# nonl4331/raytracing-rust

Measured on AMD Instinct MI355X. Metric: Msamples/s on rtweekend1.ssml 1920x1080x1024spp, higher is better.
Workload: dtype f32

## Files before the change

include/rt_hip.h:

```cpp
#ifndef RT_HIP_H
#define RT_HIP_H

#include <stdint.h>

#ifdef __cplusplus
extern "C" {
#endif

#define RT_ABI_VERSION 2u

typedef enum rt_status {
	RT_OK = 0,
	RT_ERR_INVALID_ARGUMENT = -1,
	RT_ERR_NO_DEVICE = -2,
	RT_ERR_HIP = -3,
	RT_ERR_OUT_OF_MEMORY = -4,
	RT_ERR_UNSUPPORTED = -5
} rt_status;

typedef enum rt_texture_type {
	RT_TEX_CHECKERED = 0,
	RT_TEX_SOLID = 1,
	RT_TEX_IMAGE = 2,
	RT_TEX_LERP = 3,
// ... 332 lines not shown
	float metered;
	uint32_t reserved;
} rt_display_state;
int rt_display_opts_default(rt_display_opts *out);
int rt_display_workspace_bytes(const rt_display_opts *opts, uint64_t *bytes);
int rt_display_output_bytes(const rt_display_opts *opts, uint64_t *bytes);
int rt_display_device(rt_scene *scene, const float *d_rgb, const rt_display_opts *opts, rt_display_state *d_state,
                      void *d_workspace, void *d_out, uint32_t *d_histogram, void *hip_stream);
int rt_display(rt_scene *scene, const float *host_rgb, const rt_display_opts *opts, void *host_out, rt_display_state *host_state,
               uint32_t *host_histogram);
int rt_display_reset(rt_scene *scene);

typedef struct rt_upscale_opts {
	uint32_t src_width, src_height;
	uint32_t dst_width, dst_height;
	float sigma_normal;
	float depth_tolerance;
	uint32_t reserved[8];
} rt_upscale_opts;
typedef struct rt_upscale_inputs {
	const float *color;
	const float *src_albedo, *src_normal, *src_depth;
	const float *dst_albedo, *dst_normal, *dst_depth;
} rt_upscale_inputs;
int rt_upscale_opts_default(rt_upscale_opts *out);
int rt_upscale_device(rt_scene *scene, const rt_upscale_inputs *device_in, const rt_upscale_opts *opts, float *d_out, uint8_t *d_stage,
                      void *hip_stream);
int rt_upscale(rt_scene *scene, const rt_upscale_inputs *host_in, const rt_upscale_opts *opts, float *host_out, uint8_t *host_stage);
int rt_render_upscaled(rt_scene *scene, const rt_camera *camera, const rt_render_opts *opts, uint32_t src_width, uint32_t src_height,
                       const rt_denoise_opts *dopts, const rt_upscale_opts *uopts, float *out, float *out_src, uint64_t *rays_shot);

int rt_selftest_division(float divisor, float *reciprocal, int *exact);

#define RT_SELFTEST_LEAN_CLASSES 9
int rt_selftest_lean(int device, uint64_t n_per_thread, uint64_t seed, uint64_t mismatches[RT_SELFTEST_LEAN_CLASSES]);

#ifdef __cplusplus
}
#endif
#endif
```

raytracing-rust_amd/abi.py:

```python
import ctypes as C

RT_ABI_VERSION = 2
RT_GATHER_NONE, RT_GATHER_RCCL, RT_GATHER_PEER, RT_GATHER_PEER_STAGED, RT_GATHER_SAME_DEVICE = 0, 1, 2, 3, 4

RT_OK = 0
RT_ERR_INVALID_ARGUMENT = -1
RT_ERR_NO_DEVICE = -2
RT_ERR_HIP = -3
RT_ERR_OUT_OF_MEMORY = -4
RT_ERR_UNSUPPORTED = -5

RT_TEX_CHECKERED, RT_TEX_SOLID, RT_TEX_IMAGE, RT_TEX_LERP, RT_TEX_PERLIN = range(5)
RT_MAT_EMIT, RT_MAT_LAMBERTIAN, RT_MAT_TROWBRIDGE_REITZ, RT_MAT_REFLECT, RT_MAT_REFRACT = range(5)
RT_PRIM_SPHERE, RT_PRIM_TRIANGLE, RT_PRIM_MESH_TRIANGLE = range(3)
RT_SPLIT_SAH, RT_SPLIT_MIDDLE, RT_SPLIT_EQUAL_COUNTS = range(3)
RT_METHOD_NAIVE, RT_METHOD_MIS = range(2)
RT_LAYOUT_FRAME, RT_LAYOUT_SHARD = range(2)
RT_TUNE_TRAVERSAL, RT_TUNE_FEATURE_SET, RT_TUNE_SCENE_IN_LDS, RT_TUNE_SCHEDULE, RT_TUNE_WALK, RT_TUNE_STACK_CAP, RT_TUNE_EXCHANGE = range(7)

NO_INDEX = 0xFFFFFFFFFFFFFFFF
RT_DEVICE_NONE = -1

f32x3 = C.c_float * 3

# ... 331 lines not shown
    "rt_aov_chain_buffers": (AovChainBuffers, 56),
    "rt_denoise_opts": (DenoiseOpts, 48),
    "rt_denoise_inputs": (DenoiseInputs, 40),
    "rt_temporal_opts": (TemporalOpts, 96),
    "rt_temporal_inputs": (TemporalInputs, 32),
    "rt_display_opts": (DisplayOpts, 104),
    "rt_display_state": (DisplayState, 16),
    "rt_upscale_opts": (UpscaleOpts, 56),
    "rt_upscale_inputs": (UpscaleInputs, 56),
}

EXPORTED_SYMBOLS = [
    "rt_last_error",
    "rt_abi_version",
    "rt_device_count",
    "rt_render_opts_default",
    "rt_camera_new",
    "rt_scene_create",
    "rt_scene_create_multi",
    "rt_scene_device_count",
    "rt_scene_destroy",
    "rt_scene_counts",
    "rt_scene_get_nodes",
    "rt_scene_get_primitive_order",
    "rt_scene_get_lights",
    "rt_scene_wide_info",
    "rt_scene_get_wide_nodes",
    "rt_scene_get_leaf_boxes",
    "rt_scene_get_wide_nodes_compact",
    "rt_scene_auto_sample_split",
    "rt_scene_gather_info",
    "rt_rccl_probe",
    "rt_selftest_division",
    "rt_scene_get_leaf_boxes_compact",
    "rt_scene_set_traversal",
    "rt_scene_set_tuning",
    "rt_render",
    "rt_sample_image",
    "rt_render_device",
    "rt_render_output_floats",
    "rt_shard_pixel_order",
    "rt_last_kernel_ms",
    "rt_last_launch_info",
    "rt_output_rgb8",
    "rt_output_save",
    "rt_output_rgb8_device",
    "rt_render_rgb8",
    "rt_check_hit",
    "rt_check_hit_index",
    "rt_selftest_lean",
    "rt_render_aov",
    "rt_render_aov_device",
    "rt_aov_chain_opts_default",
    "rt_render_aov_chain",
    "rt_render_aov_chain_device",
    "rt_denoise_opts_default",
    "rt_denoise_workspace_bytes",
    "rt_denoise",
    "rt_denoise_device",
    "rt_render_denoised",
    "rt_temporal_opts_default",
    "rt_temporal_history_bytes",
    "rt_temporal_workspace_bytes",
    "rt_denoise_temporal_device",
    "rt_denoise_temporal",
    "rt_denoise_temporal_reset",
# ... 42 lines not shown
```

raytracing-rust_amd/csrc/rt_api.cpp:

```cpp
#include <hip/hip_runtime.h>

#include <cstdio>
#include <cstdlib>
#include <algorithm>
#include <cmath>
#include <cstring>
#include <string>
#include <vector>

#include "../../include/rt_hip.h"
#include "../../include/rt_detmath.h"
#include <dlfcn.h>
#include "rt_api_internal.h"

namespace rt {
size_t render_lds_bytes(const DevScene &S, bool sky_lds, bool scene_lds, uint32_t waves_per_block, uint32_t stack_cap);
uint32_t render_waves_per_simd(int feature_set, bool fine);
uint32_t render_block_threads(int feature_set, bool fine, bool xchg = false);
size_t render_exchange_fine_lds_bytes(uint32_t waves_per_block);
uint32_t render_max_block_threads(int feature_set, bool fine, bool xchg);
hipError_t render_occupancy(int method, bool prune, bool fine, bool sky_lds, int feature_set, size_t lds_bytes, int *blocks_per_cu, bool xchg,
                            uint32_t block_threads = 0);
bool render_exchange_available(int method, bool prune, bool fine, int feature_set);
size_t render_exchange_lds_bytes(uint32_t slots);
// ... 1036 lines not shown
			return fail(RT_ERR_NO_DEVICE, "host-only scene");
		return render_device_multi(s, camera, o, d_out_rgb, d_rays_shot, static_cast<hipStream_t>(hip_stream));
	}
	ShardGeometry g;
	int rc = shard_geometry(o, g);
	if (rc != RT_OK)
		return rc;
	if (s->device == RT_DEVICE_NONE)
		return fail(RT_ERR_NO_DEVICE, "host-only scene (RT_DEVICE_NONE): rendering needs a GPU, there is no CPU fallback");
	if (o->render_method != RT_METHOD_NAIVE && o->render_method != RT_METHOD_MIS)
		return fail(RT_ERR_INVALID_ARGUMENT, "unknown render method");
	if (o->samples_per_pixel == 0 || o->samples_per_pixel >= (1ull << 32))
		return fail(RT_ERR_INVALID_ARGUMENT, "samples_per_pixel must be in [1, 2^32)");
	if (o->output_layout != RT_LAYOUT_FRAME && o->output_layout != RT_LAYOUT_SHARD)
		return fail(RT_ERR_INVALID_ARGUMENT, "unknown output layout");
	HIP_TRY(hipSetDevice(s->device));
	hipStream_t stream = static_cast<hipStream_t>(hip_stream);
	if (g.n_work == 0) {
		HIP_TRY(launch_reset(stream, s->d_work_counter, reinterpret_cast<unsigned long long *>(d_rays_shot), d_out_rgb,
		                     o->output_layout == RT_LAYOUT_FRAME ? (size_t)(o->width * o->height * 3) : 0));
		s->timed = false;
		return RT_OK;
	}

	DevRenderParams P;
	std::memset(&P, 0, sizeof P);
	P.width = (uint32_t)o->width;
	P.height = (uint32_t)o->height;
	P.spp = (uint32_t)o->samples_per_pixel;
	P.sample_begin_lo = (uint32_t)o->sample_begin;
	P.sample_begin_hi = (uint32_t)(o->sample_begin >> 32);
	P.seed_lo = (uint32_t)o->seed;
	P.seed_hi = (uint32_t)(o->seed >> 32);
	P.max_depth = o->max_depth;
	P.rr_threshold = o->rr_threshold;
	P.shard_index = o->shard_index;
	P.shard_count = o->shard_count;
	P.tile_w = g.tile_w;
	P.tile_h = g.tile_h;
	P.tiles_x = g.tiles_x;
	P.tiles_y = g.tiles_y;
	P.n_work = (uint32_t)g.n_work;
	uint32_t split = o->sample_split;
	if (split == 0u)
		split = auto_sample_split(s->n_cus, o->width * o->height, o->samples_per_pixel, o->shard_count);
	{
		float rw = 0.0f, rh = 0.0f;
		const bool sized = o->width <= (1u << 24) && o->height <= (1u << 24);
		const bool ok_w = sized && verified_reciprocal((float)(o->width - 1), &rw), ok_h = sized && verified_reciprocal((float)(o->height - 1), &rh);
		const bool ok = ok_w && ok_h;
		P.w1h1_ok = ok ? 1u : 0u;
		P.inv_w1 = rw;
		P.inv_h1 = rh;
	}
	P.tile_log2_w = 0xFFFFFFFFu;
	if (g.tile_w * g.tile_h == 64u && (g.tile_w & (g.tile_w - 1u)) == 0u && o->width < 65536u && o->height < 65536u &&
	    (split & (split - 1u)) == 0u && split <= 64u)
		for (uint32_t lw = 0; lw < 7u; ++lw)
			for (uint32_t ls = 0; ls < 7u; ++ls)
				if ((1u << lw) == g.tile_w && (1u << ls) == split)
					P.tile_log2_w = lw | (ls << 8);
	if (split > o->samples_per_pixel)
		return fail(RT_ERR_INVALID_ARGUMENT, "sample_split larger than samples_per_pixel");
	if (g.n_work * split >= (1ull << 32))
		return fail(RT_ERR_UNSUPPORTED, "pixels x sample_split exceeds 2^32 work items");
	P.sample_split = split;
// ... 645 lines not shown
	DevScene dev = s->dev;
	const bool walks_wide = prune && dev.nodes4 != nullptr && dev.narrow_only == 0u;
	if (!walks_wide || (size_t)4 * dev.stack_depth * 64u * sizeof(uint32_t) > s->max_lds) {
		if (walks_wide)
			dev.narrow_only = 1u;
		dev.stack_depth = s->stack_depth_narrow;
	}
	if (e == hipSuccess)
		e = object_index ? launch_check_hit_index(prune, s->stream, dev, d_rays, d_idx, n, d_out)
		                 : launch_check_hit(prune, s->stream, dev, d_rays, n, d_out);
	if (e == hipSuccess)
		e = hipMemcpyAsync(out, d_out, n * sizeof(rt_hit_record), hipMemcpyDeviceToHost, s->stream);
	if (e == hipSuccess)
		e = hipStreamSynchronize(s->stream);
	(void)hipFree(d_rays);
	(void)hipFree(d_out);
	(void)hipFree(d_idx);
	if (e != hipSuccess)
		return hip_fail(e, "check_hit");
	return RT_OK;
}

int rt_check_hit(rt_scene *s, const rt_ray_desc *rays, uint64_t n_rays, rt_hit_record *out)
{
	return check_common(s, rays, nullptr, n_rays, out);
}
int rt_check_hit_index(rt_scene *s, const rt_ray_desc *rays, const uint64_t *object_index, uint64_t n_rays, rt_hit_record *out)
{
	if (!object_index)
		return fail(RT_ERR_INVALID_ARGUMENT, "null argument");
	return check_common(s, rays, object_index, n_rays, out);
}

int rt_selftest_division(float divisor, float *reciprocal, int *exact)
{
	if (!reciprocal || !exact)
		return fail(RT_ERR_INVALID_ARGUMENT, "null argument");
	*exact = verified_reciprocal(divisor, reciprocal) ? 1 : 0;
	return RT_OK;
}

int rt_selftest_lean(int device, uint64_t n_per_thread, uint64_t seed, uint64_t mismatches[RT_SELFTEST_LEAN_CLASSES])
{
	if (!mismatches || n_per_thread == 0 || n_per_thread > (1ull << 20))
		return fail(RT_ERR_INVALID_ARGUMENT, "bad arguments (n_per_thread in [1, 2^20])");
	int n_dev = 0;
	if (hipGetDeviceCount(&n_dev) != hipSuccess || device < 0 || device >= n_dev)
		return fail(RT_ERR_NO_DEVICE, "no such HIP device");
	HIP_TRY(hipSetDevice(device));
	unsigned long long *d = nullptr;
	HIP_TRY(hipMalloc(reinterpret_cast<void **>(&d), RT_SELFTEST_LEAN_CLASSES * sizeof(unsigned long long)));
	hipError_t e = hipMemset(d, 0, RT_SELFTEST_LEAN_CLASSES * sizeof(unsigned long long));
	if (e == hipSuccess)
		e = launch_selftest_lean(nullptr, 1024u, n_per_thread, seed, d);
	if (e == hipSuccess)
		e = hipMemcpy(mismatches, d, RT_SELFTEST_LEAN_CLASSES * sizeof(unsigned long long), hipMemcpyDeviceToHost);
	(void)hipFree(d);
	if (e != hipSuccess)
		return hip_fail(e, "selftest");
	return RT_OK;
}

}
```

raytracing-rust_amd/csrc/rt_lean.h:

```cpp
#pragma once

#include "rt_vec.h"

namespace rt {


RT_FN void lean_sincos(float x, float &s, float &c)
{
	const float k = rintf(x * 0.636619746685028076172f);
	float r = fmaf(-k, 1.57079637050628662109f, x);
	r = fmaf(-k, -4.37113882867379282984e-08f, r);
	r = fmaf(-k, -1.71512451000588185479e-15f, r);
	const int q = (int)k;
	const float sk = rt_sin_kernel(r), ck = rt_cos_kernel(r);
	const bool odd = (q & 1) != 0;
	const float sv = odd ? ck : sk;
	const float cv = odd ? sk : ck;
	s = (q & 2) ? -sv : sv;
	c = ((q + 1) & 2) ? -cv : cv;
}

RT_FN float lean_acos_with(float x, float sqrt_half_one_minus_abs)
{
	const bool big = fabsf(x) > 0.5f;
	const float k = rt_asin_kernel(big ? sqrt_half_one_minus_abs : x);
	const float two_k = 2.0f * k;
	return big ? (x > 0.0f ? two_k : RT_PI - two_k) : RT_FRAC_PI_2 - k;
}
RT_FN float lean_acos(float x) { return lean_acos_with(x, sqrtf(0.5f * (1.0f - fabsf(x)))); }

RT_FN float lean_atan_unit_with(float t, float q)
{
	const bool upper = t > 0.414213567972183227539f;
	const float u = upper ? q : t;
	const float z = u * u;
	float p = fmaf(8.05374449538e-2f, z, -1.38776856032e-1f);
	p = fmaf(p, z, 1.99777106478e-1f);
	p = fmaf(p, z, -3.33329491539e-1f);
// ... 104 lines not shown
```

raytracing-rust_amd/csrc/rt_render.hip:

```cpp
#include "rt_shade.h"

namespace rt {

enum : int {
	PH_GEN = 0,
	PH_NODE = 1,
	PH_LEAF = 2,
	PH_SHADE = 3,
	PH_LIGHT = 4,
	PH_SCATTER = 5,
	PH_NARROW = 6,
	PH_COUNT = 7,
	PH_NEED_PIXEL = 7,
	PH_DONE = 8,
	PH_WALK = 9
};

#ifndef RT_PQ_SPLIT
#define RT_PQ_SPLIT 1
#endif
#ifndef RT_LIGHT_PHASE_THRESHOLD
#define RT_LIGHT_PHASE_THRESHOLD 48
#endif
constexpr uint32_t kLightPhaseThreshold = RT_LIGHT_PHASE_THRESHOLD;
// ... 31 lines not shown
#define RT_SIMPLE_COARSE_WAVES 5
#endif
#ifndef RT_SIMPLE_COARSE_BLOCK
#define RT_SIMPLE_COARSE_BLOCK 256
#endif
#ifndef RT_SPHERES_BLOCK
#define RT_SPHERES_BLOCK 512
#endif
#ifndef RT_FUSE_REGIONS
#define RT_FUSE_REGIONS(spheres_only) true
#endif
#ifndef RT_BODY_ALWAYS
#define RT_BODY_ALWAYS(spheres_only) true
#endif
#ifndef RT_SPHERES_MAX_BLOCK
#define RT_SPHERES_MAX_BLOCK 768
#endif
#ifndef RT_PAIR_WAVES
#define RT_PAIR_WAVES 6
#endif
#ifndef RT_SPHERES_WAVES
#define RT_SPHERES_WAVES 4
#endif
#ifndef RT_SPHERES_COARSE_WAVES
#define RT_SPHERES_COARSE_WAVES 6
#endif

__device__ __forceinline__ float power_heuristic(float pdf_a, float pdf_b)
{
	const float a_sq = pdf_a * pdf_a;
	return a_sq / (a_sq + pdf_b * pdf_b);
}

__device__ __forceinline__ bool work_to_pixel(const DevRenderParams &P, uint32_t w, uint32_t &x, uint32_t &y)
{
	const uint32_t tile_pixels = P.tile_w * P.tile_h;
	const uint32_t k = w / tile_pixels;
	const uint32_t in = w - k * tile_pixels;
	const uint32_t tile = P.shard_index + k * P.shard_count;
	const uint32_t ty = tile / P.tiles_x;
	const uint32_t tx = tile - ty * P.tiles_x;
	x = tx * P.tile_w + in % P.tile_w;
	y = ty * P.tile_h + in / P.tile_w;
	return x < P.width && y < P.height;
}

template <class F, bool FINE = false, bool XCHG = false> struct KernelShape {
	static constexpr bool spheres_only = !(F::tri || F::lights || F::cmat || F::ctex);
	static constexpr bool simple = !spheres_only && !(F::cmat || F::ctex);
	static constexpr int waves_per_simd = (F::cmat || F::ctex) ? (FINE ? RT_FULL_FINE_WAVES : (XCHG ? 3 : RT_FULL_WAVES))
	                                      : (F::pair ? RT_PAIR_WAVES : (spheres_only ? ((FINE || XCHG) ? RT_SPHERES_WAVES : RT_SPHERES_COARSE_WAVES)
	                                                                                 : (FINE ? RT_SIMPLE_FINE_WAVES : (XCHG ? 4 : RT_SIMPLE_COARSE_WAVES))));
	static constexpr int block = (FINE && XCHG) ? 512 : (spheres_only ? RT_SPHERES_BLOCK : ((simple && !FINE) ? RT_SIMPLE_COARSE_BLOCK : 256));
	static constexpr int max_block = ((spheres_only || simple) && !FINE && !XCHG && block == 512) ? RT_SPHERES_MAX_BLOCK : block;
};

#ifdef RT_STATS
#define RT_SECTION(k) do { const unsigned long long now_ = wall_clock64(); st_sect[(k)] += now_ - st_mark; st_mark = now_; } while (0)
#else
#define RT_SECTION(k) do { } while (0)
#endif
#ifdef RT_STATS
__device__ unsigned long long g_stats[64];
__device__ unsigned long long g_hist[4][65];
#endif

constexpr uint32_t kXchgBStride = 44, kXchgPStride = 12;
constexpr uint32_t kXchgMaxSlots = 64;
constexpr uint32_t kXchgMinLanes = 4;
constexpr uint32_t kXchgRecWords = 60;
constexpr uint32_t kXchgFineSlots = 64;
constexpr uint32_t kXchgFineHdr = 8 + 2 * 64;
#ifndef RT_XCHG_SHADERS
#define RT_XCHG_SHADERS 1
#endif
constexpr uint32_t kXchgShaderWaves = RT_XCHG_SHADERS;
enum : uint32_t { XS_EMPTY = 0, XS_FULL = 1, XS_BUSY = 2 };

struct RenderArgs {
	DevScene S;
	DevCamera cam;
	DevRenderParams P;
	float *out;
	unsigned long long *rays_shot;
	uint32_t *work_counter;
	uint32_t *stack_ovf;
	DevPairScene pair;
};
#if defined(__HIP_DEVICE_COMPILE__)
typedef const __attribute__((address_space(4))) RenderArgs *KArgs;
#else
typedef const RenderArgs *KArgs;
#endif
// ... 190 lines not shown
			ph = any_hit ? PH_SCATTER : PH_SHADE;
		else
			ph = ref_is_leaf(node) ? PH_LEAF : PH_NODE;
	};
	auto finalize = [&](bool filter) {
		V3 c = outp;
		if (filter && (contains_nan(c) || !is_finite_any(c)))
			c = v3s(0.0f);
		if (P.sample_split > 1u) {
			mean.x += c.x;
			mean.y += c.y;
			mean.z += c.z;
		} else {
			const float i_f = (float)(sample_local + 1u);
			mean.x += (c.x - mean.x) / i_f;
			mean.y += (c.y - mean.y) / i_f;
			mean.z += (c.z - mean.z) / i_f;
		}
		rays_total += ray_count;
		sample_local += 1;
		if (sample_local == chunk_n) {
			float *const out = kargs()->out;
			out[3u * (size_t)out_index + 0u] = mean.x;
			out[3u * (size_t)out_index + 1u] = mean.y;
			out[3u * (size_t)out_index + 2u] = mean.z;
			ph = PH_NEED_PIXEL;
		} else {
			ph = PH_GEN;
		}
	};

	auto do_gen = [&]() {
		const KArgs k = kargs();
		const uint64_t seed = ((uint64_t)k->P.seed_hi << 32) | k->P.seed_lo;
		const uint64_t sample_begin = ((uint64_t)k->P.sample_begin_hi << 32) | k->P.sample_begin_lo;
		const V3 cam_o = v3(k->cam.origin[0], k->cam.origin[1], k->cam.origin[2]);
		const V3 cam_ll = v3(k->cam.lower_left[0], k->cam.lower_left[1], k->cam.lower_left[2]);
		const V3 cam_h = v3(k->cam.horizontal[0], k->cam.horizontal[1], k->cam.horizontal[2]);
		const V3 cam_v = v3(k->cam.vertical[0], k->cam.vertical[1], k->cam.vertical[2]);
		const uint32_t w1 = here_(k->P.width - 1u), h1 = here_(k->P.height - 1u);
		rt_rng_seed(&rng, seed, (uint64_t)pixel_index, sample_begin + chunk_begin + sample_local);
		RT_SECTION(15);
		const float jx = rt_rng_range_f32(&rng, 0.0f, 1.0f) + (float)px, jy = rt_rng_range_f32(&rng, 0.0f, 1.0f) + (float)py;
		float u, v;
		if (here_(k->P.w1h1_ok) != 0u) {
			u = div_by_verified(jx, (float)w1, k->P.inv_w1);
			v = 1.0f - div_by_verified(jy, (float)h1, k->P.inv_h1);
		} else {
			u = div_tame_fix_(jx, (float)w1);
			v = 1.0f - div_tame_fix_(jy, (float)h1);
		}
		ray = ray_new<F>(cam_o, cam_ll + cam_h * u + cam_v * v - cam_o);
		(void)rt_rng_f32(&rng);
		thr = v3s(1.0f);
		outp = v3s(0.0f);
		depth = 0;
		ray_count = 0;
		primary = true;
		begin_walk(false);
	
	};

#ifdef RT_STATS
	unsigned long long st_lane_nodes = 0, st_lane_prims = 0, st_lane_maxsp = 0;
#endif
	auto do_node = [&]() {
#ifdef RT_STATS
		st_lane_nodes += 1;
		if ((unsigned long long)sp > st_lane_maxsp)
			st_lane_maxsp = (unsigned long long)sp;
#endif
		const bool limit_valid = any_hit ? !(PL.t_limit != PL.t_limit) : (best_prim != kNoPrim);
		if (SM.ovf_depth == 0u)
			node = descend4<PRUNE, false>(S, SM, ray, node, stk, sp, limit_valid, any_hit ? PL.t_limit : best_t);
// ... 101 lines not shown
			}
		} else if (arm == 1 || (arm == 0 && primary)) {
			wo = ray.d;
			hit = nh;
			mat = nmat;
			RT_SECTION(13);
			const V3 emission = emission_of_hit<F>(S, PS, mat, prim == kNoPrim, hit, wo);
			Ray clone = ray;
			const bool exit = mat_scatter_ray<F>(S, mat, clone, hit, rng, known_new);
			outp = outp + emission;
			RT_SECTION(14);
			if (exit) {
				finish = true;
				filter = false;
			} else {
				depth = 1;
				primary = false;
				if (!(depth < P.max_depth))
					finish = true;
			}
		} else {
			const V3 m_wi = ray.d;
			const float m_pdf = mat_scattering_pdf<F>(S, mat, hit, wo, m_wi, known_path);
			const V3 le = emission_of_hit<F>(S, PS, nmat, prim == kNoPrim, hit , m_wi);
			thr = thr * mat_eval_over_pdf<F>(S, mat, hit, wo, m_wi, known_path, PS);
			RT_SECTION(11);
			if (!is_zero(le)) {
				const bool on_light = F::lights && (prim != kNoPrim) && mat_is_light(S, nmat) && !mat_is_delta<F>(S, mat);
				if (on_light || (prim == kNoPrim && sky_samplable)) {
					const uint32_t n_l = F::lights ? S.n_lights : 0u;
					const uint32_t n_choices = sky_samplable ? n_l + 1u : n_l;
					float l_pdf;
					if (prim == kNoPrim) {
						l_pdf = div_by_count(sky_pdf(S, T, m_wi), n_choices);
					} else {
						const PrimGeom g = load_prim<F>(S, prim);
						l_pdf = div_by_count(prim_scattering_pdf<F>(g, hit.point, m_wi, nh), n_choices);
					}
					const float mis_weight = power_heuristic(m_pdf, l_pdf);
					outp = outp + thr * le * mis_weight;
				} else {
					outp = outp + thr * le;
				}
			}
			RT_SECTION(12);
			if (mat_is_light<F>(S, nmat, known_new)) {
				finish = true;
			} else {
				if (depth > P.rr_threshold) {
					const float p = component_max(thr);
					if (rt_rng_f32(&rng) > p)
						finish = true;
					else
						thr = thr / p;
				}
				if (!finish) {
					wo = m_wi;
					hit = nh;
					mat = nmat;
					depth += 1;
					if (!(depth < P.max_depth))
						finish = true;
				}
			}
		}
		if (finish)
			finalize(filter);
// ... 43 lines not shown
				g = load_prim_uniform<F>(&S_global.prims[L.skip]);
			} else {
				L.skip = S.lights[light_slot];
				g = load_prim<F>(S, L.skip);
			}
			L.l_wi = prim_sample_visible_from_point<F>(g, hit.point, rng);
		}
		if (pick_sky || pick_light)
			sr = ray_new<F>(shadow_origin, L.l_wi);
		if (pick_light) {
			float lt;
			if (prim_t<F>(g, sr, lt) && lt > 0.0f) {
				L.t_limit = lt;
				L.have_shadow = true;
			}
		}
		if (L.have_shadow) {
			begin_walk(true);
		} else {
			best_prim = kNoPrim;
			ph = PH_SCATTER;
		}
	
	};

	auto do_scatter = [&](LightCtx &L, Ray &sr) {
		const bool occluded = best_prim != kNoPrim;
		if (L.have_shadow && !occluded) {
			bool valid = false;
			V3 le = v3s(0.0f);
			float l_pdf = 0.0f;
			if (L.shadow_is_sky) {
				le = emission_of_hit<F>(S, PS, S.sky.material, true, hit, L.l_wi);
				l_pdf = sky_pdf(S, T, L.l_wi) * L.pdf_multiplier;
				valid = true;
			} else {
				Hit lh;
				uint32_t lm;
				PrimGeom g;
				if (S.single_light != kNoPrim) {
					g = load_prim_uniform<F>(&S_global.prims[L.skip]);
					if (!F::tri || g.type == kPrimSphere) {
						make_sphere_hit_by_reciprocal(g.p0, g.p1.x, g.p1.y, sr, L.t_limit, lh);
						lm = g.material;
					} else {
						make_hit<F>(S, L.skip, sr, L.t_limit, lh, lm);
					}
				} else {
					make_hit<F>(S, L.skip, sr, L.t_limit, lh, lm);
					g = load_prim<F>(S, L.skip);
				}
				const float p = prim_scattering_pdf<F>(g, hit.point, L.l_wi, lh);
				if (p > 0.0f) {
					le = mat_get_emission<F>(S, lm, lh, L.l_wi);
					l_pdf = p * L.pdf_multiplier;
					valid = true;
				}
			}
			if (valid) {
				const float m_pdf = mat_scattering_pdf<F>(S, mat, hit, wo, L.l_wi, known_path);
				const float mis_weight = power_heuristic(l_pdf, m_pdf);
				outp = outp + thr * mat_eval<F>(S, mat, hit, wo, L.l_wi, known_path, PS) * mis_weight * le / l_pdf;
			}
		}
		RT_SECTION(10);
		ray.d = wo;
		if (mat_scatter_ray<F>(S, mat, ray, hit, rng, known_path))
// ... 516 lines not shown
			} else if (run == PH_LEAF) {
				if (ph == PH_LEAF)
					do_leaf();
			} else if (run == PH_GEN) {
				if (ph == PH_GEN)
					do_gen();
			} else if (run == PH_SHADE) {
				if (ph == PH_SHADE)
					do_shade(std::integral_constant<int, 0>{});
			} else if (run == PH_LIGHT) {
				if (ph == PH_LIGHT)
					do_light(PL, ray);
			} else if (run == PH_NARROW) {
				if (ph == PH_NARROW)
					do_narrow();
			} else {
				if (ph == PH_SCATTER)
					do_scatter(PL, ray);
			}
#ifdef RT_STATS
			if (lane == 0u) {
				const unsigned long long now_ = wall_clock64();
				st_fine_clock[run] += now_ - st_mark;
				st_mark = now_;
			}
#endif
		}
	}

	if constexpr (!FINE) {
		bool alive = true;
		uint32_t waited = 0;
		while (alive) {
			if (XCHG && METHOD == 1)
				exchange();
			acquire();
			const uint32_t n_light = (uint32_t)__popcll(__ballot(ph == PH_LIGHT));
			const uint32_t n_trace = (METHOD == 1 && RT_PQ_SPLIT) ? (uint32_t)__popcll(__ballot(ph == PH_GEN))
			                                                      : (uint32_t)__popcll(__ballot(ph == PH_GEN || ph == PH_NODE || ph == PH_LEAF || ph == PH_SHADE));
			constexpr bool kBodyAlways = RT_BODY_ALWAYS(KernelShape<F>::spheres_only);
			if (kBodyAlways) {
				alive = (n_light + n_trace != 0u) || __ballot(ph == PH_NEED_PIXEL) != 0ull;
				if (XCHG && METHOD == 1 && !alive)
					alive = __hip_atomic_load(&pool[1], __ATOMIC_RELAXED, __HIP_MEMORY_SCOPE_WORKGROUP) != 0u ||
					        __hip_atomic_load(&pool[2], __ATOMIC_RELAXED, __HIP_MEMORY_SCOPE_WORKGROUP) != 0u;
			}
			if (kBodyAlways || n_light + n_trace != 0u) {
				const bool run_light = (METHOD == 1) && (n_light >= kLightPhaseThreshold || n_trace == 0u || (kStarveLimit != 0u && waited >= kStarveLimit));
				waited = run_light ? 0u : waited + n_light;
	#ifdef RT_STATS
				if (lane == 0u) {
					if (!run_light) {
						st_iters[0] += 1; st_active[0] += n_trace;
						st_hist[((n_trace ? n_trace : 1u) - 1u) >> 3] += 1;
#ifndef RT_STATS_NO_HIST
						atomicAdd(&g_hist[0][n_trace], 1ull);
						atomicAdd(&g_hist[1][n_light], 1ull);
#endif
						st_gen += (unsigned long long)__popcll(__ballot(ph == PH_GEN));
					} else {
						st_iters[1] += 1; st_active[1] += n_light;
#ifndef RT_STATS_NO_HIST
						atomicAdd(&g_hist[3][n_light], 1ull);
#endif
					}
				}
	#endif
				RT_SECTION(0);
				constexpr bool kFuseRegions = METHOD == 1 && RT_PQ_SPLIT && RT_FUSE_REGIONS(KernelShape<F>::spheres_only);
// ... 54 lines not shown
								do_shade(std::integral_constant<int, 2>{});
							}
						}
						RT_SECTION(8);
					} else {
						load_pair_scene();
						if (ph == PH_LIGHT)
							do_light(L, sray);
						RT_SECTION(4);
						walk_shadow_pending(L, sray);
						RT_SECTION(5);
						if (ph == PH_SCATTER)
							do_scatter(L, sray);
						RT_SECTION(6);
	#if RT_PQ_SPLIT
						walk_closest_pending();
						RT_SECTION(7);
						if (ph == PH_SHADE)
							do_shade(std::integral_constant<int, 2>{});
						RT_SECTION(8);
	#endif
					}
				}
	#if RT_PQ_SPLIT
				if (METHOD == 1) {
					ray.o = ray.d = ray.inv = ray.shear = v3s(0.0f);
					best_t = 0.0f;
					best_prim = kNoPrim;
					node = kRefDone;
					sp = 0;
					any_hit = false;
				}
	#endif
			} else {
				alive = __ballot(ph == PH_NEED_PIXEL) != 0ull;
				if (XCHG && METHOD == 1)
					alive = alive || __hip_atomic_load(&pool[1], __ATOMIC_RELAXED, __HIP_MEMORY_SCOPE_WORKGROUP) != 0u ||
					        __hip_atomic_load(&pool[2], __ATOMIC_RELAXED, __HIP_MEMORY_SCOPE_WORKGROUP) != 0u;
			}
		}
	}
#ifdef RT_STATS
	atomicAdd(&g_stats[20], st_lane_nodes);
	atomicAdd(&g_stats[21], st_lane_prims);
	atomicMax(&g_stats[22], st_lane_maxsp);
	if (lane == 0u) {
		for (int k = 0; k < 9; ++k)
			atomicAdd(&g_stats[40 + k], st_sect[k]);
		if (!FINE)
			for (int k = 9; k < 16; ++k)
				atomicAdd(&g_stats[40 + k], st_sect[k]);
		for (int k = 0; k < 8; ++k)
			atomicAdd(&g_stats[24 + k], st_hist[k]);
		for (int k = 0; k <= PH_COUNT; ++k)
			atomicAdd(&g_stats[50 + k], st_fine_clock[k]);
		atomicAdd(&g_stats[0], st_iters[0]); atomicAdd(&g_stats[1], st_active[0]);
		atomicAdd(&g_stats[2], st_iters[1]); atomicAdd(&g_stats[3], st_active[1]);
		atomicAdd(&g_stats[4], st_gen);
		for (int k = 0; k < PH_COUNT; ++k) {
			atomicAdd(&g_stats[5 + k], st_fine_iters[k]);
			atomicAdd(&g_stats[5 + PH_COUNT + k], st_fine_active[k]);
		}
	}
#endif
	unsigned long long *const rays_shot = K->rays_shot;
	if (rays_shot != nullptr) {
// ... 649 lines not shown
```

raytracing-rust_amd/csrc/rt_shade.h:

```cpp
#pragma once

#include "rt_intersect.h"

namespace rt {

__device__ __forceinline__ float sqrt_unit_(float x)
{
#if defined(__HIP_DEVICE_COMPILE__) && !defined(RT_NO_LEAN)
	return lean_sqrt(x);
#else
	return sqrtf(x);
#endif
}
__device__ __forceinline__ float div_tame_fix_(float n, float d)
{
#if defined(__HIP_DEVICE_COMPILE__) && !defined(RT_NO_LEAN)
	return lean_div_fix(n, d);
#else
	return n / d;
#endif
}

__device__ __forceinline__ float next_float(float f)
{
// ... 43 lines not shown
	Coord c;
	if (fabsf(z.x) > fabsf(z.y))
		c.x = v3(-z.z, 0.0f, z.x) / sqrtf(z.x * z.x + z.z * z.z);
	else
		c.x = v3(0.0f, z.z, -z.y) / sqrtf(z.y * z.y + z.z * z.z);
	c.y = cross(c.x, z);
	c.z = z;
	return c;
}
__device__ __forceinline__ Coord coord_from_z_zsel(V3 z)
{
	Coord c;
	if (fabsf(z.x) > fabsf(z.y)) {
		const float s = sqrtf(z.x * z.x + z.z * z.z);
		c.x = v3(-z.z / s, s > 0.0f ? 0.0f : __builtin_nanf(""), z.x / s);
	} else {
		const float s = sqrtf(z.y * z.y + z.z * z.z);
		c.x = v3(s > 0.0f ? 0.0f : __builtin_nanf(""), z.z / s, -z.y / s);
	}
	c.y = cross(c.x, z);
	c.z = z;
	return c;
}
__device__ __forceinline__ Coord coord_inverse(const Coord &c)
{
	Coord r;
	r.x = v3(c.x.x, c.y.x, c.z.x);
	r.y = v3(c.x.y, c.y.y, c.z.y);
	r.z = v3(c.x.z, c.y.z, c.z.z);
	return r;
}
__device__ __forceinline__ V3 to_coord(const Coord &c, V3 v) { return v.x * c.x + v.y * c.y + v.z * c.z; }

__device__ __forceinline__ uint32_t f32_as_index(float f)
{
	if (!(f > 0.0f))
		return 0u;
	if (f >= 4294967040.0f)
		return 0xFFFFFFFFu;
	return (uint32_t)f;
}
__device__ __forceinline__ int32_t f32_as_i32(float f)
{
	if (f != f)
		return 0;
	if (f >= 2147483648.0f)
		return 2147483647;
	if (f <= -2147483648.0f)
		return (-2147483647 - 1);
	return (int32_t)f;
}

__device__ inline float perlin_noise(const DevTexture &t, V3 point)
{
	const float u = point.x - floorf(point.x);
	const float v = point.y - floorf(point.y);
	const float w = point.z - floorf(point.z);
	const int32_t i = f32_as_i32(floorf(point.x));
	const int32_t j = f32_as_i32(floorf(point.y));
	const int32_t k = f32_as_i32(floorf(point.z));
	const float uu = u * u * (3.0f - 2.0f * u);
	const float vv = v * v * (3.0f - 2.0f * v);
	const float ww = w * w * (3.0f - 2.0f * w);
	float value = 0.0f;
	for (int index = 0; index < 8; ++index) {
		const int ii = index / 4, jj = (index / 2) % 2, kk = index % 2;
		const uint32_t a = t.perlin_perm[(uint32_t)(i + ii) & 255u] ^ t.perlin_perm[256 + ((uint32_t)(j + jj) & 255u)] ^
		                   t.perlin_perm[512 + ((uint32_t)(k + kk) & 255u)];
		const float *rv = t.perlin_vecs + 3 * (a & 255u);
		const V3 c = v3(rv[0], rv[1], rv[2]);
		const float fi = (float)ii, fj = (float)jj, fk = (float)kk;
		const V3 weight = v3(u - fi, v - fj, w - fk);
		value += (fi * uu + (1.0f - fi) * (1.0f - uu)) * (fj * vv + (1.0f - fj) * (1.0f - vv)) *
		         (fk * ww + (1.0f - fk) * (1.0f - ww)) * dot(c, weight);
	}
	return value;
}

template <class F> __device__ __forceinline__ V3 texture_colour(const DevScene &S, uint32_t tex, V3 direction, V3 point)
{
	const DevTexture &t = S.textures[tex];
	const int type = t.type;
	if (type == 1)
		return v3(t.c1[0], t.c1[1], t.c1[2]);
	if (type == 3) {
		const float tt = direction.z * 0.5f + 0.5f;
		return v3(t.c1[0], t.c1[1], t.c1[2]) * tt + v3(t.c2[0], t.c2[1], t.c2[2]) * (1.0f - tt);
	}
	if (!F::ctex)
		return v3s(1.0f);
	if (type == 0) {
		const float sign = rt_sinf(10.0f * point.x) * rt_sinf(10.0f * point.y) * rt_sinf(10.0f * point.z);
		return sign > 0.0f ? v3(t.c1[0], t.c1[1], t.c1[2]) : v3(t.c2[0], t.c2[1], t.c2[2]);
	}
	if (type == 2) {
		const float phi = lean_atan2(direction.y, direction.x) + kPi;
		const float theta = lean_acos_dev(direction.z);
		const float uvx = phi / (2.0f * kPi);
		const float uvy = theta / kPi;
		const uint32_t x_pixel = f32_as_index((float)t.dim_x * uvx);
		const uint32_t y_pixel = f32_as_index((float)t.dim_y * uvy);
		uint64_t index = (uint64_t)y_pixel * (t.dim_x + 1u) + x_pixel;
		const uint64_t n = (uint64_t)(t.dim_x + 1u) * (t.dim_y + 1u);
		if (index >= n)
			index = n - 1;
		const float *px = t.image + 3 * index;
		return v3(px[0], px[1], px[2]);
	}
	if (type == 4)
		return (0.5f * v3s(1.0f)) * (1.0f + perlin_noise(t, point));
	return v3s(1.0f);
}

enum : int { kMatRead = -1, kMatEmit = 0, kMatLambertian = 1 };
template <class F> __device__ __forceinline__ int mat_type_(uint32_t mat, int known)
{
	if (F::known_materials && known != kMatRead)
		return known;
	return mat_handle_type(mat);
}
__device__ __forceinline__ const DevMaterial &mat_record(const DevScene &S, uint32_t mat) { return S.materials[mat_handle_index(mat)]; }

template <class F> __device__ __forceinline__ V3 material_texture_colour(const DevScene &S, const DevMaterial &m, uint32_t mat, V3 direction, V3 point)
{
	const int type = mat_handle_tex_type(mat);
	if (type == 1)
		return v3(m.tex_c1[0], m.tex_c1[1], m.tex_c1[2]);
	if (type == 3) {
		const float tt = direction.z * 0.5f + 0.5f;
		return v3(m.tex_c1[0], m.tex_c1[1], m.tex_c1[2]) * tt + v3(m.tex_c2[0], m.tex_c2[1], m.tex_c2[2]) * (1.0f - tt);
	}
	if (!F::ctex)
		return v3s(1.0f);
	return texture_colour<F>(S, m.texture, direction, point);
// ... 49 lines not shown
	} else {
		first = 0;
		uint32_t len = n + 1;
		while (len > 0) {
			const uint32_t half = len >> 1;
			const uint32_t middle = first + half;
			if (cdf[middle] <= num) {
				first = middle + 1;
				len -= half + 1;
			} else {
				len = half;
			}
		}
	}
	const uint32_t v = first - 1u;
	return v > n - 1u ? n - 1u : v;
}

#if defined(__HIP_DEVICE_COMPILE__)
typedef const __attribute__((address_space(4))) uint32_t *KWords;
#else
typedef const uint32_t *KWords;
#endif
struct SkyTables {
	const float *row_cdf;
	const float *marginal_cdf;
	const uint8_t *guide;
	uint32_t guide_k;
	KWords inv_res;
};

__device__ __forceinline__ bool sky_can_sample(const DevScene &S) { return (S.sky.res_x | S.sky.res_y) != 0u; }

__device__ __forceinline__ float sky_pdf(const DevScene &S, const SkyTables &T, V3 wi)
{
	const float sin_theta = sqrt_unit_(1.0f - wi.z * wi.z);
	if (sin_theta <= 0.0f)
		return 0.0f;
	const float theta = lean_acos_dev(wi.z);
	float phi = lean_atan2(wi.y, wi.x);
	if (phi < 0.0f)
		phi += 2.0f * kPi;
	const float u = div_by_verified(phi, kTau, kRcpTau);
	const float v = div_by_verified(theta, kPi, kRcpPi);
	const uint32_t rx = here_(S.sky.res_x), ry = here_(S.sky.res_y);
	uint32_t ui = f32_as_index((float)rx * u);
	uint32_t vi = f32_as_index((float)ry * v);
	ui = ui > rx - 1u ? rx - 1u : ui;
	vi = vi > ry - 1u ? ry - 1u : vi;
	const float ypdf = T.marginal_cdf[vi + 1u] - T.marginal_cdf[vi];
	const float *row = T.row_cdf + (size_t)vi * (rx + 1u);
	const float xpdf = row[ui + 1u] - row[ui];
	return (float)rx * (float)ry * (ypdf * xpdf) / (sin_theta * kTau * kPi);
}

__device__ __forceinline__ V3 sky_sample(const DevScene &S, const SkyTables &T, rt_rng &rng)
{
	const uint32_t rx = here_(S.sky.res_x), ry = here_(S.sky.res_y);
	const bool guided = T.guide_k != 0u;
	const uint32_t sv = dist1d_sample(T.marginal_cdf, ry, guided ? T.guide + (size_t)ry * T.guide_k : nullptr, T.guide_k, rng);
	const uint32_t su = dist1d_sample(T.row_cdf + (size_t)sv * (rx + 1u), rx, guided ? T.guide + (size_t)sv * T.guide_k : nullptr, T.guide_k, rng);
	const float nu = next_float((float)su + rt_rng_f32(&rng)), nv = next_float((float)sv + rt_rng_f32(&rng));
	float u, v;
	KWords inv = T.inv_res;
#if defined(__HIP_DEVICE_COMPILE__)
	asm volatile("" : "+s"(inv));
#endif
	if (inv != nullptr && inv[0] != 0u) {
		u = div_by_verified(nu, (float)rx, __uint_as_float(inv[1]));
		v = div_by_verified(nv, (float)ry, __uint_as_float(inv[2]));
	} else {
		u = nu / (float)rx;
		v = nv / (float)ry;
	}
	const float phi = u * 2.0f * kPi;
	const float theta = v * kPi;
	float st, ct, sp, cp;
	lean_sincos(theta, st, ct);
	lean_sincos(phi, sp, cp);
	return v3(st * cp, st * sp, ct);
// ... 336 lines not shown
```

raytracing-rust_amd/csrc/rt_types.h:

```cpp
#pragma once

#include <stdint.h>
#include "rt_vec.h"

namespace rt {

constexpr uint32_t kNoPrim = 0xFFFFFFFFu;

template <bool TRI, bool LIGHTS, bool CMAT, bool CTEX> struct Feat {
	static constexpr bool tri = TRI;
	static constexpr bool lights = LIGHTS;
	static constexpr bool cmat = CMAT;
	static constexpr bool ctex = CTEX;
	static constexpr bool pair = false;
	static constexpr bool known_materials = false;
};
using FeatFull = Feat<true, true, true, true>;
struct FeatPair : Feat<false, false, false, false> {
	static constexpr bool pair = true;
	static constexpr bool known_materials = true;
};

constexpr uint32_t kLeafFlag = 0x80000000u;
constexpr uint32_t kLeafInlineMax = 31u;
// ... 115 lines not shown
	int32_t sky_tex_type;
	float sky_c1[3], sky_c2[3];
	float inv_radius[2];
	uint32_t pad[6];
};
static_assert(sizeof(DevPairScene) == 192, "DevPairScene: three 64-byte lines");
__device__ static const DevPairScene kNoPairScene = {};

struct DevCamera {
	float origin[3], lower_left[3], horizontal[3], vertical[3];
};

struct DevRenderParams {
	uint32_t width, height;
	uint32_t spp;
	uint32_t sample_begin_lo, sample_begin_hi;
	uint32_t seed_lo, seed_hi;
	uint32_t max_depth, rr_threshold;
	uint32_t shard_index, shard_count;
	uint32_t tile_w, tile_h, tiles_x, tiles_y;
	uint32_t n_work;
	uint32_t sample_split;
	uint32_t n_items;
	int32_t shard_layout;
	int32_t prune;
	uint32_t sky_in_lds;
	uint32_t scene_in_lds;
	uint32_t stack_cap;
	uint32_t stack_ovf_depth;
	uint32_t xchg_slots;
	uint32_t tile_log2_w;
	uint32_t w1h1_ok;
	float inv_w1, inv_h1;
};

}
```

raytracing-rust_amd/hip_backend.py:

```python
import ctypes as C
import os
import sys

import numpy as np

from . import abi

_HERE = os.path.dirname(os.path.abspath(__file__))
LIB_PATH = os.environ.get("RT_HIP_LIB") or os.path.join(_HERE, "librt_hip.so")
_LIB = None


class RtHipError(RuntimeError):
    def __init__(self, code, message):
        super().__init__(f"rt_hip error {code}: {message}")
        self.code = code


def lib():
    global _LIB
    if _LIB is None:
        if not os.path.exists(LIB_PATH):
            raise RtHipError(abi.RT_ERR_NO_DEVICE, f"{LIB_PATH} not built (run `make -C raytracing-rust_amd/csrc`); "
                             "the HIP back end has no CPU fallback")
# ... 22 lines not shown


def _set_f32_inputs(ins, color, optional, keep):
    color = np.ascontiguousarray(color, dtype=np.float32)
    if color.ndim != 3 or color.shape[2] != 3:
        raise ValueError(f"color must be (H, W, 3), got {color.shape}")
    h, w = color.shape[:2]
    keep.append(color)
    ins.color = _p(color, C.c_float)
    for name, a, channels in optional:
        if a is None:
            continue
        shape = (h, w, channels) if channels > 1 else (h, w)
        a = np.ascontiguousarray(a, dtype=np.float32)
        if a.shape != shape:
            raise ValueError(f"{name} must be {shape}, got {a.shape}")
        keep.append(a)
        setattr(ins, name, _p(a, C.c_float))
    return h, w


def _f3(v):
    return (C.c_float * 3)(*[float(np.float32(x)) for x in v])


def rccl_probe():
    usable, note = C.c_int(), C.create_string_buffer(512)
    _check(lib().rt_rccl_probe(C.byref(usable), note, C.c_uint64(512)))
    return bool(usable.value), note.value.decode()


def device_count():
    return int(lib().rt_device_count())


def selftest_lean(device=0, n_per_thread=64, seed=1):
    out = (C.c_uint64 * 9)()
    _check(lib().rt_selftest_lean(C.c_int(device), C.c_uint64(n_per_thread), C.c_uint64(seed), out))
    return [int(x) for x in out]


def camera_new(origin, lookat, vup, fov, aspect_ratio, aperture, focus_dist):
    cam = abi.Camera()
    _check(lib().rt_camera_new(C.byref(cam), _f3(origin), _f3(lookat), _f3(vup), C.c_float(fov),
                               C.c_float(aspect_ratio), C.c_float(aperture), C.c_float(focus_dist)))
    return cam


HIT_DTYPE = np.dtype([("t", "<f4"), ("point", "<f4", 3), ("error", "<f4", 3), ("normal", "<f4", 3), ("uv", "<f4", 2),
                      ("has_uv", "<i4"), ("out", "<i4"), ("material", "<u4"), ("found", "<u4"), ("index", "<u8")])
NODE_DTYPE = np.dtype([("min", "<f4", 3), ("max", "<f4", 3), ("children", "<i8", 2), ("primitive_offset", "<u8"),
                       ("number_primitives", "<u8")])


WIDE_NODE_DTYPE = np.dtype([("origin", "<f4", 3), ("exps", "<u4"), ("qlo", "<u4", 3), ("qhi", "<u4", 3), ("child", "<u4", 4),
                            ("pad", "<u4", 2)])


def _pack_rays(origins, directions):
    o = np.asarray(origins, dtype=np.float32).reshape(-1, 3)
    d = np.asarray(directions, dtype=np.float32).reshape(-1, 3)
    return np.ascontiguousarray(np.concatenate([o, d], axis=1))


class HipScene:

# ... 532 lines not shown
```

Measured before the change: 36670.

## Precompute Philox round keys on host and pass them via render params

Computes the ten Philox-4x32 round key pairs on the host from the seed, stores them in DevRenderParams, and seeds the per-sample RNG on the non-fine path from the loaded keys. This removes the per-thread key-schedule additions. It also templates sky_pdf so that spheres-only kernels use a select-based float-to-index cast instead of a branchy one, and adds optional s_nop census markers. The risks are extra kernel-argument loads (20 words) and higher register pressure from holding the key array.

```diff
diff --git a/include/rt_hip.h b/include/rt_hip.h
--- a/include/rt_hip.h
+++ b/include/rt_hip.h
@@ -388,6 +388,8 @@
 
 int rt_selftest_division(float divisor, float *reciprocal, int *exact);
 
+int rt_philox_round_keys(uint64_t seed, uint32_t keys[20]);
+
 #define RT_SELFTEST_LEAN_CLASSES 9
 int rt_selftest_lean(int device, uint64_t n_per_thread, uint64_t seed, uint64_t mismatches[RT_SELFTEST_LEAN_CLASSES]);
 
diff --git a/raytracing-rust_amd/abi.py b/raytracing-rust_amd/abi.py
--- a/raytracing-rust_amd/abi.py
+++ b/raytracing-rust_amd/abi.py
@@ -387,6 +387,7 @@
     "rt_scene_gather_info",
     "rt_rccl_probe",
     "rt_selftest_division",
+    "rt_philox_round_keys",
     "rt_scene_get_leaf_boxes_compact",
     "rt_scene_set_traversal",
     "rt_scene_set_tuning",
diff --git a/raytracing-rust_amd/csrc/rt_api.cpp b/raytracing-rust_amd/csrc/rt_api.cpp
--- a/raytracing-rust_amd/csrc/rt_api.cpp
+++ b/raytracing-rust_amd/csrc/rt_api.cpp
@@ -1092,6 +1092,7 @@
 	P.sample_begin_hi = (uint32_t)(o->sample_begin >> 32);
 	P.seed_lo = (uint32_t)o->seed;
 	P.seed_hi = (uint32_t)(o->seed >> 32);
+	philox_round_keys(o->seed, P.philox_key);
 	P.max_depth = o->max_depth;
 	P.rr_threshold = o->rr_threshold;
 	P.shard_index = o->shard_index;
@@ -1803,6 +1804,14 @@
 	return check_common(s, rays, object_index, n_rays, out);
 }
 
+int rt_philox_round_keys(uint64_t seed, uint32_t keys[20])
+{
+	if (!keys)
+		return fail(RT_ERR_INVALID_ARGUMENT, "null argument");
+	philox_round_keys(seed, keys);
+	return RT_OK;
+}
+
 int rt_selftest_division(float divisor, float *reciprocal, int *exact)
 {
 	if (!reciprocal || !exact)
diff --git a/raytracing-rust_amd/csrc/rt_lean.h b/raytracing-rust_amd/csrc/rt_lean.h
--- a/raytracing-rust_amd/csrc/rt_lean.h
+++ b/raytracing-rust_amd/csrc/rt_lean.h
@@ -4,6 +4,20 @@
 
 namespace rt {
 
+
+RT_FN uint32_t f32_as_index_branchy(float f)
+{
+	if (!(f > 0.0f))
+		return 0u;
+	if (f >= 4294967040.0f)
+		return 0xFFFFFFFFu;
+	return (uint32_t)f;
+}
+RT_FN uint32_t f32_as_index(float f)
+{
+	const uint32_t r = (uint32_t)fmin_(fmax_(f, 0.0f), 4294967040.0f);
+	return f >= 4294967040.0f ? 0xFFFFFFFFu : r;
+}
 
 RT_FN void lean_sincos(float x, float &s, float &c)
 {
diff --git a/raytracing-rust_amd/csrc/rt_render.hip b/raytracing-rust_amd/csrc/rt_render.hip
--- a/raytracing-rust_amd/csrc/rt_render.hip
+++ b/raytracing-rust_amd/csrc/rt_render.hip
@@ -87,6 +87,30 @@
 	return a_sq / (a_sq + pdf_b * pdf_b);
 }
 
+__device__ __forceinline__ void rng_seed_keyed(rt_rng *r, const uint32_t (&rk)[20], uint64_t pixel, uint64_t sample)
+{
+	uint32_t c[4] = {(uint32_t)pixel, (uint32_t)(pixel >> 32), (uint32_t)sample, (uint32_t)(sample >> 32)};
+#pragma unroll
+	for (int round = 0; round < 10; ++round) {
+		const uint64_t p0 = (uint64_t)0xD2511F53u * (uint64_t)c[0];
+		const uint64_t p1 = (uint64_t)0xCD9E8D57u * (uint64_t)c[2];
+		const uint32_t hi0 = (uint32_t)(p0 >> 32), lo0 = (uint32_t)p0;
+		const uint32_t hi1 = (uint32_t)(p1 >> 32), lo1 = (uint32_t)p1;
+		const uint32_t n0 = hi1 ^ c[1] ^ rk[2 * round];
+		const uint32_t n2 = hi0 ^ c[3] ^ rk[2 * round + 1];
+		c[0] = n0;
+		c[1] = lo1;
+		c[2] = n2;
+		c[3] = lo0;
+	}
+	if ((c[0] | c[1] | c[2] | c[3]) == 0u)
+		c[0] = 1u;
+	r->s0 = c[0];
+	r->s1 = c[1];
+	r->s2 = c[2];
+	r->s3 = c[3];
+}
+
 __device__ __forceinline__ bool work_to_pixel(const DevRenderParams &P, uint32_t w, uint32_t &x, uint32_t &y)
 {
 	const uint32_t tile_pixels = P.tile_w * P.tile_h;
@@ -112,8 +136,13 @@
 
 #ifdef RT_STATS
 #define RT_SECTION(k) do { const unsigned long long now_ = wall_clock64(); st_sect[(k)] += now_ - st_mark; st_mark = now_; } while (0)
+#define RT_LOOP_MARK(k) do { } while (0)
+#elif defined(RT_CENSUS_MARKS)
+#define RT_SECTION(k) asm volatile("s_nop %0" ::"n"(0x40 + (k)))
+#define RT_LOOP_MARK(k) asm volatile("s_nop %0" ::"n"(0x40 + (k)))
 #else
 #define RT_SECTION(k) do { } while (0)
+#define RT_LOOP_MARK(k) do { } while (0)
 #endif
 #ifdef RT_STATS
 __device__ unsigned long long g_stats[64];
@@ -370,14 +399,25 @@
 
 	auto do_gen = [&]() {
 		const KArgs k = kargs();
-		const uint64_t seed = ((uint64_t)k->P.seed_hi << 32) | k->P.seed_lo;
+		uint32_t rk[20] = {};
+		uint64_t seed = 0;
+		if constexpr (FINE) {
+			seed = ((uint64_t)k->P.seed_hi << 32) | k->P.seed_lo;
+		} else {
+#pragma unroll
+			for (int i = 0; i < 20; ++i)
+				rk[i] = k->P.philox_key[i];
+		}
 		const uint64_t sample_begin = ((uint64_t)k->P.sample_begin_hi << 32) | k->P.sample_begin_lo;
 		const V3 cam_o = v3(k->cam.origin[0], k->cam.origin[1], k->cam.origin[2]);
 		const V3 cam_ll = v3(k->cam.lower_left[0], k->cam.lower_left[1], k->cam.lower_left[2]);
 		const V3 cam_h = v3(k->cam.horizontal[0], k->cam.horizontal[1], k->cam.horizontal[2]);
 		const V3 cam_v = v3(k->cam.vertical[0], k->cam.vertical[1], k->cam.vertical[2]);
 		const uint32_t w1 = here_(k->P.width - 1u), h1 = here_(k->P.height - 1u);
-		rt_rng_seed(&rng, seed, (uint64_t)pixel_index, sample_begin + chunk_begin + sample_local);
+		if constexpr (FINE)
+			rt_rng_seed(&rng, seed, (uint64_t)pixel_index, sample_begin + chunk_begin + sample_local);
+		else
+			rng_seed_keyed(&rng, rk, (uint64_t)pixel_index, sample_begin + chunk_begin + sample_local);
 		RT_SECTION(15);
 		const float jx = rt_rng_range_f32(&rng, 0.0f, 1.0f) + (float)px, jy = rt_rng_range_f32(&rng, 0.0f, 1.0f) + (float)py;
 		float u, v;
@@ -545,7 +585,7 @@
 					const uint32_t n_choices = sky_samplable ? n_l + 1u : n_l;
 					float l_pdf;
 					if (prim == kNoPrim) {
-						l_pdf = div_by_count(sky_pdf(S, T, m_wi), n_choices);
+						l_pdf = div_by_count(sky_pdf<KernelShape<F>::spheres_only>(S, T, m_wi), n_choices);
 					} else {
 						const PrimGeom g = load_prim<F>(S, prim);
 						l_pdf = div_by_count(prim_scattering_pdf<F>(g, hit.point, m_wi, nh), n_choices);
@@ -655,7 +695,7 @@
 			float l_pdf = 0.0f;
 			if (L.shadow_is_sky) {
 				le = emission_of_hit<F>(S, PS, S.sky.material, true, hit, L.l_wi);
-				l_pdf = sky_pdf(S, T, L.l_wi) * L.pdf_multiplier;
+				l_pdf = sky_pdf<KernelShape<F>::spheres_only>(S, T, L.l_wi) * L.pdf_multiplier;
 				valid = true;
 			} else {
 				Hit lh;
@@ -1238,9 +1278,11 @@
 		bool alive = true;
 		uint32_t waited = 0;
 		while (alive) {
+			RT_LOOP_MARK(16);
 			if (XCHG && METHOD == 1)
 				exchange();
 			acquire();
+			RT_LOOP_MARK(18);
 			const uint32_t n_light = (uint32_t)__popcll(__ballot(ph == PH_LIGHT));
 			const uint32_t n_trace = (METHOD == 1 && RT_PQ_SPLIT) ? (uint32_t)__popcll(__ballot(ph == PH_GEN))
 			                                                      : (uint32_t)__popcll(__ballot(ph == PH_GEN || ph == PH_NODE || ph == PH_LEAF || ph == PH_SHADE));
@@ -1361,6 +1403,7 @@
 					any_hit = false;
 				}
 	#endif
+				RT_LOOP_MARK(17);
 			} else {
 				alive = __ballot(ph == PH_NEED_PIXEL) != 0ull;
 				if (XCHG && METHOD == 1)
diff --git a/raytracing-rust_amd/csrc/rt_shade.h b/raytracing-rust_amd/csrc/rt_shade.h
--- a/raytracing-rust_amd/csrc/rt_shade.h
+++ b/raytracing-rust_amd/csrc/rt_shade.h
@@ -99,14 +99,6 @@
 }
 __device__ __forceinline__ V3 to_coord(const Coord &c, V3 v) { return v.x * c.x + v.y * c.y + v.z * c.z; }
 
-__device__ __forceinline__ uint32_t f32_as_index(float f)
-{
-	if (!(f > 0.0f))
-		return 0u;
-	if (f >= 4294967040.0f)
-		return 0xFFFFFFFFu;
-	return (uint32_t)f;
-}
 __device__ __forceinline__ int32_t f32_as_i32(float f)
 {
 	if (f != f)
@@ -165,8 +157,8 @@
 		const float theta = lean_acos_dev(direction.z);
 		const float uvx = phi / (2.0f * kPi);
 		const float uvy = theta / kPi;
-		const uint32_t x_pixel = f32_as_index((float)t.dim_x * uvx);
-		const uint32_t y_pixel = f32_as_index((float)t.dim_y * uvy);
+		const uint32_t x_pixel = f32_as_index_branchy((float)t.dim_x * uvx);
+		const uint32_t y_pixel = f32_as_index_branchy((float)t.dim_y * uvy);
 		uint64_t index = (uint64_t)y_pixel * (t.dim_x + 1u) + x_pixel;
 		const uint64_t n = (uint64_t)(t.dim_x + 1u) * (t.dim_y + 1u);
 		if (index >= n)
@@ -282,6 +274,7 @@
 
 __device__ __forceinline__ bool sky_can_sample(const DevScene &S) { return (S.sky.res_x | S.sky.res_y) != 0u; }
 
+template <bool SELECT_CAST>
 __device__ __forceinline__ float sky_pdf(const DevScene &S, const SkyTables &T, V3 wi)
 {
 	const float sin_theta = sqrt_unit_(1.0f - wi.z * wi.z);
@@ -294,8 +287,8 @@
 	const float u = div_by_verified(phi, kTau, kRcpTau);
 	const float v = div_by_verified(theta, kPi, kRcpPi);
 	const uint32_t rx = here_(S.sky.res_x), ry = here_(S.sky.res_y);
-	uint32_t ui = f32_as_index((float)rx * u);
-	uint32_t vi = f32_as_index((float)ry * v);
+	uint32_t ui = SELECT_CAST ? f32_as_index((float)rx * u) : f32_as_index_branchy((float)rx * u);
+	uint32_t vi = SELECT_CAST ? f32_as_index((float)ry * v) : f32_as_index_branchy((float)ry * v);
 	ui = ui > rx - 1u ? rx - 1u : ui;
 	vi = vi > ry - 1u ? ry - 1u : vi;
 	const float ypdf = T.marginal_cdf[vi + 1u] - T.marginal_cdf[vi];
diff --git a/raytracing-rust_amd/csrc/rt_types.h b/raytracing-rust_amd/csrc/rt_types.h
--- a/raytracing-rust_amd/csrc/rt_types.h
+++ b/raytracing-rust_amd/csrc/rt_types.h
@@ -171,6 +171,18 @@
 	uint32_t tile_log2_w;
 	uint32_t w1h1_ok;
 	float inv_w1, inv_h1;
+	uint32_t philox_key[20];
 };
 
+inline void philox_round_keys(uint64_t seed, uint32_t keys[20])
+{
+	uint32_t k0 = (uint32_t)seed, k1 = (uint32_t)(seed >> 32);
+	for (int round = 0; round < 10; ++round) {
+		keys[2 * round] = k0;
+		keys[2 * round + 1] = k1;
+		k0 += 0x9E3779B9u;
+		k1 += 0xBB67AE85u;
+	}
 }
+
+}
diff --git a/raytracing-rust_amd/hip_backend.py b/raytracing-rust_amd/hip_backend.py
--- a/raytracing-rust_amd/hip_backend.py
+++ b/raytracing-rust_amd/hip_backend.py
@@ -78,6 +78,12 @@
 
 def device_count():
     return int(lib().rt_device_count())
+
+
+def philox_round_keys(seed):
+    out = (C.c_uint32 * 20)()
+    _check(lib().rt_philox_round_keys(C.c_uint64(seed), out))
+    return [int(x) for x in out]
 
 
 def selftest_lean(device=0, n_per_thread=64, seed=1):
```

Result: slower. 36260 (-1.1%).
